# aask1357/hilcodec

Measured on AMD Instinct MI355X. Metric: audio-seconds/sec (xRT) encode+RVQ+decode, 24 kHz batch=256, higher is better.
Workload: dtype f32

## Files before the change

hilcodec_amd/csrc/resblock_kernel.h:

```cpp
#pragma once
#include "resblock_gemm.h"
#include "stream_gemm.h"

namespace {

struct Cols {
  long b;
  int t;
  int t_in;
  unsigned boff;
  unsigned hoff;
  int head, tail;
};
static_assert(sizeof(Cols) == 32, "no padding");

template <int C, bool STREAM, bool SCARRY = false, int NB = 1, bool W8 = false, int DRU = 0, bool POST = false, bool SPEC0 = false>
__global__ __launch_bounds__((Cfg<C, STREAM, SCARRY, NB, W8, DRU, POST, SPEC0>::NT), (Cfg<C, STREAM, SCARRY, NB, W8, DRU, POST, SPEC0>::MINW)) void resblock_kernel(ResArgs a) {
  using K = Cfg<C, STREAM, SCARRY, NB, W8, DRU, POST, SPEC0>;
  constexpr int DR = K::DR, UR = K::UR;
  using Pipe = WeightPipe<K>;
  constexpr int CBW = K::CBW, NW = K::NW, NT = K::NT, RW = K::RW, RB = K::RB, XS = K::XS, TO = K::TO, RSTEP = K::RSTEP;
  __shared__ __attribute__((aligned(16))) float Xbuf[4 + C * XS];
  constexpr bool DW_RELOAD = NB > 1 && K::NARROW && (4 + C * XS + NB * C * DWS) * 4 > 156 * 1024;
  __shared__ __attribute__((aligned(16))) float DW[(DW_RELOAD ? 1 : NB) * C * DWS];
// ... 80 lines not shown
      }
    } else {
    float tv[NB][RND][DWS];
#pragma unroll
    for (int q = 0; q < NB; ++q) {
      if (q < nblk) {
        const ResBlk& bq = a.blk[q];
#pragma unroll
        for (int it = 0; it < RND; ++it) {
          const int m = tid + it * NT;
          const int mc = (C % NT == 0 || m < C) ? m : C - 1;
#pragma unroll
          for (int j = 0; j < 5; ++j) tv[q][it][j] = bq.dw1_w[mc * 5 + j];
          tv[q][it][5] = bq.dw1_b[mc];
#pragma unroll
          for (int j = 0; j < 5; ++j) tv[q][it][6 + j] = bq.dw2_w[mc * 5 + j];
          tv[q][it][11] = bq.dw2_b[mc];
        }
      }
    }
#pragma unroll
    for (int q = 0; q < NB; ++q) {
      if (q < nblk) {
#pragma unroll
        for (int it = 0; it < RND; ++it) {
          const int m = tid + it * NT;
          if (C % NT == 0 || m < C) {
#pragma unroll
            for (int w4 = 0; w4 < DWS / 4; ++w4)
              *reinterpret_cast<f32x4*>(&DW[(q * C + m) * DWS + 4 * w4]) =
                  f32x4{tv[q][it][4 * w4], tv[q][it][4 * w4 + 1], tv[q][it][4 * w4 + 2], tv[q][it][4 * w4 + 3]};
          }
        }
      }
    }
    }
  }
  if constexpr (DR > 0 && !DWIDE) {
    constexpr int RND = (2 * C + NT - 1) / NT;
    float tw[RND][2 * DR + 1];
#pragma unroll
    for (int it = 0; it < RND; ++it) {
      const int m = tid + it * NT;
      const int mc = ((2 * C) % NT == 0 || m < 2 * C) ? m : 2 * C - 1;
#pragma unroll
      for (int j = 0; j < 2 * DR; ++j) tw[it][j] = a.dn.dw_w[mc * 2 * DR + j];
      tw[it][2 * DR] = a.dn.dw_b[mc];
    }
#pragma unroll
    for (int it = 0; it < RND; ++it) {
      const int m = tid + it * NT;
      if ((2 * C) % NT == 0 || m < 2 * C) {
#pragma unroll
        for (int j = 0; j < DDS; ++j) DWD[m * DDS + j] = j < 2 * DR ? tw[it][j] : (j == 8 ? tw[it][2 * DR] : 0.f);
      }
    }
  }
  if (tid < 4) Xbuf[tid] = 0.f;
  const int rsub = wave * K::RPI + (K::RPI > 1 ? lane / (K::NCOL / 4) : 0);
  const int c4 = (lane & (K::NCOL / 4 - 1)) * 4;
  [[maybe_unused]] const unsigned row_b = (unsigned)T * 4u;
  [[maybe_unused]] const bool one_head = STREAM && !K::NARROW && T >= K::NCOL;

  auto columns_of = [&](long tile) -> Cols {
    Cols s;
    s.boff = 0; s.hoff = 0; s.head = false; s.tail = false;
    if constexpr (STREAM) {
      const int flat = (int)tile * TO - K::HALO + c4;
      s.t_in = flat >= 0 && flat < a.B * T;
      const unsigned ub = s.t_in ? __umulhi((unsigned)flat, a.div_magic) >> a.div_shift : 0u;
      s.b = ub;
      s.t = s.t_in ? flat - (int)ub * T : 0;
      s.boff = (ub * (unsigned)(C * T) + (unsigned)s.t) * 4u;
      s.hoff = ub * (unsigned)(C * 4);
      s.head = s.t_in && s.t == 0;
      s.tail = s.t_in && c4 >= K::HALO && s.t == T - 4;
    } else {
      s.b = tile / a.tiles;
      s.t = (int)(tile - s.b * a.tiles) * TO + c4;
      s.t_in = s.t >= 0 && s.t < T;
    }
    return s;
  };
  auto xrow = [&](const Cols& s, int m) -> const f32x4* {
    if constexpr (STREAM)
      return reinterpret_cast<const f32x4*>(reinterpret_cast<const char*>(a.x) + (s.boff + (unsigned)m * row_b));
    else
      return reinterpret_cast<const f32x4*>(a.x + s.b * (long)C * T + (long)m * T + (s.t_in ? s.t : 0));
  };
  auto yrow = [&](const Cols& s, int m) -> f32x4* {
    if constexpr (STREAM)
      return reinterpret_cast<f32x4*>(reinterpret_cast<char*>(a.y) + (s.boff + (unsigned)m * row_b));
    else
      return reinterpret_cast<f32x4*>(a.y + s.b * (long)C * T + (long)m * T + s.t);
  };

  [[maybe_unused]] const float* hb0 = a.x;
  [[maybe_unused]] const float* hb1 = a.x;
  [[maybe_unused]] bool hv0 = false, hv1 = false;
  [[maybe_unused]] int blk_off = 0;
  Cols cs;
  const bool lane0 = c4 == 0, lane_last = c4 == K::NCOL - 4;
  auto prev_base = [&](int which) -> lptr_t {
    if constexpr (!K::CARRYMODE) return (lptr_t)(X + rsub * XS + c4 - 4);
    else return lane0 ? (lptr_t)(X + rsub * XS + K::NCOL + which * 4 + blk_off) : (lptr_t)(X + rsub * XS + c4 - 4);
  };
  auto prevs_of = [&](lptr_t pb, int m0, int which, f32x4 (&prev)[K::RB]) {
    if constexpr (!STREAM) {
#pragma unroll
      for (int i = 0; i < K::RB; ++i) prev[i] = *(lvec_t)(pb + i * RSTEP * XS);
    } else {
      bool staged = false;
      if constexpr (!K::NARROW) staged = one_head;
      if (staged) {
#pragma unroll
        for (int i = 0; i < K::RB; ++i) {
          const lptr_t pa = cs.head ? (lptr_t)(HS + (which * C + m0 + RSTEP * i) * 4) : pb + i * RSTEP * XS;
          prev[i] = *(lvec_t)pa;
        }
      } else {
        f32x4 hv[K::RB];
#pragma unroll
        for (int i = 0; i < K::RB; ++i)
          hv[i] = *reinterpret_cast<const f32x4*>((which ? hb1 : hb0) + ((which ? hv1 : hv0) ? cs.hoff + (unsigned)(m0 + RSTEP * i) * 4u : 0u));
#pragma unroll
        for (int i = 0; i < K::RB; ++i) {
          const f32x4 own = *(lvec_t)(pb + i * RSTEP * XS);
#pragma unroll
          for (int e = 0; e < 4; ++e) prev[i][e] = cs.head ? ((which ? hv1 : hv0) ? hv[i][e] : 0.f) : own[e];
        }
      }
    }
  };
  auto carry_out = [&](lptr_t xp, int which, const f32x4 (&cur)[K::RB]) {
    if constexpr (K::CARRYMODE) {
      if (lane_last) {
#pragma unroll
        for (int i = 0; i < K::RB; ++i) *(lvec_t)(xp + i * RSTEP * XS + 4 + which * 4 + blk_off) = cur[i];
      }
    }
  };

  float touch = 0.f;
  constexpr int LPR = K::NCOL / 32;
#ifdef HILC_RES_NO_UTOUCH
  constexpr bool UTOUCH = false;
#else
  constexpr bool UTOUCH = !STREAM && UR > 0 && !K::NARROW && (K::NCOL / (UR > 0 ? UR : 1)) % 32 == 0;
#endif
  constexpr int LPRU = UTOUCH ? K::NCOL / UR / 32 : 1;
  constexpr int NTOUCH = STREAM ? 1 : (UTOUCH ? (2 * C * LPRU + NT - 1) / NT : (C * LPR + NT - 1) / NT);
  float tv[NTOUCH];
#pragma unroll
  for (int i = 0; i < NTOUCH; ++i) tv[i] = 0.f;
  __shared__ long s_next;
  long run0 = blockIdx.x, run1 = a.total_tiles;
  long tile = blockIdx.x;
  if constexpr (K::CARRYMODE) {
    if (a.classes > 1) {
      const unsigned P = gridDim.x / (unsigned)a.classes, u = blockIdx.x % P, c = blockIdx.x / P;
      const long s0 = (long)u * a.total_tiles / P, len = (long)(u + 1) * a.total_tiles / P - s0;
      run0 = s0 + ((len * (long)a.cum[c]) >> 16);
      run1 = s0 + ((len * (long)a.cum[c + 1]) >> 16);
    } else if (a.run_tiles > 0) {
      run0 = (long)blockIdx.x * a.run_tiles;
      run1 = run0 + a.run_tiles < a.total_tiles ? run0 + a.run_tiles : a.total_tiles;
    } else {
      run0 = (long)blockIdx.x * a.total_tiles / gridDim.x;
      run1 = ((long)blockIdx.x + 1) * a.total_tiles / gridDim.x;
    }
    const bool mid = STREAM ? (run0 * TO) % T != 0 : run0 % a.tiles != 0;
    tile = (mid && run0 < run1) ? run0 - 1 : run0;
  }
  cs = columns_of(tile < run1 ? tile : 0);
  f32x4 xr[RW];
  if (UR == 0 && !SPEC0 && tile < run1) {
#pragma unroll
    for (int i = 0; i < RW; ++i) xr[i] = *xrow(cs, rsub + RSTEP * i);
  }
  lds_barrier();
  while (tile < run1) {
    const bool warm = K::CARRYMODE && tile < run0;
    constexpr bool TICKETS = !K::CARRYMODE && K::NW == 4;
    if constexpr (K::CARRYMODE && !STREAM) {
      if (tile % a.tiles == 0) {
        constexpr int NSLOT = 2 * NB + K::DCAR / 2 + (POST ? 1 : 0);
        for (int e = tid; e < NSLOT * C; e += NT)
          *reinterpret_cast<f32x4*>(X + (e / NSLOT) * XS + K::NCOL + (e % NSLOT) * 4) = f32x4{0.f, 0.f, 0.f, 0.f};
      }
    }
    if constexpr (!K::CARRYMODE) {
      if (TICKETS && a.sched != nullptr && tid == 0) s_next = (long)gridDim.x + atomicAdd(a.sched, 1);
    }
#if defined(HILC_DEBUG_WAVE_STAMPS)
    if (a.dbg != nullptr) {
      if (ws_base != nullptr && lane == 0) ws_base[(WS_MAXB - 1) * 3 + 1] = (unsigned long long)ws_k;
      ws_base = a.dbg + ((tile * NW + wave) * (long)WS_MAXB) * 3;
      if (lane == 0) { ws_base[(WS_MAXB - 1) * 3] = blockIdx.x; ws_base[(WS_MAXB - 1) * 3 + 2] = __builtin_amdgcn_s_memtime(); }
    }
    ws_k = 0;
#elif defined(HILC_DEBUG_STAMPS)
    stamp_tile = tile;
#endif
    STAMP(0);
    long next_tile = K::CARRYMODE ? tile + 1 : tile + gridDim.x;
    if constexpr (UR > 0) {
      const ResUp& up = a.up;
      const int Tin = T / UR;
      const int q0 = cs.t / UR, p0 = cs.t - q0 * UR;
      f32x16 acc[CBW];
#pragma unroll
      for (int i = 0; i < CBW; ++i)
#pragma unroll
        for (int r = 0; r < 16; ++r) acc[i][r] = 0.f;
#pragma nounroll
      for (int h = 0; h < 2; ++h) {
        const float* wu = (h ? up.w_hi : up.w_lo) + (long)wclass * (C * C / K::RH);
        asm volatile("" : "+s"(wu));
        {
          constexpr int UB = RW % 6 == 0 ? 6 : RB;
          constexpr bool UEXP = UR == 5;
          lptr_t xp = (lptr_t)(X + rsub * XS + c4);
          const bool has_prev = cs.t_in && q0 >= 1;
          [[maybe_unused]] const bool has_next = cs.t_in && q0 + 1 < Tin;
#pragma unroll
          for (int i0 = 0; i0 < RW; i0 += UB) {
            float xc[UB], xq[UB];
            [[maybe_unused]] float xn[UB];
            f32x4 wa[UB];
            [[maybe_unused]] f32x4 wb[UB];
#pragma unroll
            for (int i = 0; i < UB; ++i) {
              const int k = h * C + rsub + RSTEP * (i0 + i);
              const long row = (long)cs.b * (2 * C) + k;
              const float* xi = up.xin + (cs.t_in ? row * Tin + q0 : 0);
              xc[i] = xi[0];
              const float* pp = has_prev ? xi - 1 : (up.hist != nullptr && cs.t_in ? up.hist + row : xi);
              xq[i] = pp[0];
              if constexpr (UR == 2) {
                xn[i] = xi[cs.t_in ? 1 : 0];
                wa[i] = *reinterpret_cast<const f32x4*>(up.tr_w + k * 4);
              } else if constexpr (UEXP) {
                xn[i] = xi[has_next ? 1 : 0];
                const float* tw = up.tr_w + ((long)k * UR + p0) * 8;
                wa[i] = *reinterpret_cast<const f32x4*>(tw);
                wb[i] = *reinterpret_cast<const f32x4*>(tw + 4);
              } else {
                wa[i] = *reinterpret_cast<const f32x4*>(up.tr_w + k * (2 * UR) + p0);
                wb[i] = *reinterpret_cast<const f32x4*>(up.tr_w + k * (2 * UR) + UR + p0);
              }
            }
#pragma unroll
            for (int i = 0; i < UB; ++i) {
              const float a1 = prologue(xc[i], up.in_scale, 1);
              const float a0 = has_prev ? prologue(xq[i], up.in_scale, 1) : (up.hist != nullptr ? xq[i] : 0.f);
              f32x4 u;
              float a_last = a1;
              if constexpr (UR == 2) {
                const float a2 = prologue(xn[i], up.in_scale, 1);
                u[0] = fmaf(wa[i].x, a1, wa[i].z * a0);
                u[1] = fmaf(wa[i].y, a1, wa[i].w * a0);
                u[2] = fmaf(wa[i].x, a2, wa[i].z * a1);
                u[3] = fmaf(wa[i].y, a2, wa[i].w * a1);
                a_last = a2;
              } else if constexpr (UEXP) {
                const float a2 = has_next ? prologue(xn[i], up.in_scale, 1) : 0.f;
#pragma unroll
                for (int e = 0; e < 4; ++e) {
                  const bool nx = p0 + e >= UR;
                  u[e] = fmaf(wa[i][e], nx ? a2 : a1, wb[i][e] * (nx ? a1 : a0));
                }
                a_last = p0 + 3 >= UR ? a2 : a1;
              } else {
#pragma unroll
                for (int e = 0; e < 4; ++e) u[e] = fmaf(wa[i][e], a1, wb[i][e] * a0);
              }
              *(lvec_t)(xp + i * RSTEP * XS) = zero_unless(cs.t_in, u);
              if constexpr (STREAM) {
                if (cs.tail && !warm && up.hist_out != nullptr)
                  up.hist_out[(long)cs.b * (2 * C) + h * C + rsub + RSTEP * (i0 + i)] = a_last;
              }
            }
            xp += UB * RSTEP * XS;
            asm volatile("" : "+v"(xp));
            __builtin_amdgcn_sched_barrier(0);
          }
        }
        Pipe wp;
        wp.prefetch(wu, lane);
        lds_barrier();
        if constexpr (K::NARROW) gemm_phase_rolled<K, false>(wu, X, acc, wp, colblk, lane);
        else gemm_phase<K, false>(wu, X, acc, wp, colblk, lane);
        lds_barrier();
      }
      acc_to_x<K>(acc, X, rowblk0, colblk, lane);
      lds_barrier();
      {
        lptr_t xp = (lptr_t)(X + rsub * XS + c4);
#pragma unroll
        for (int i = 0; i < RW; ++i) {
          const float bv = up.bias != nullptr ? up.bias[rsub + RSTEP * i] : 0.f;
          f32x4 v = *(lvec_t)(xp + i * RSTEP * XS);
#pragma unroll
          for (int e = 0; e < 4; ++e) v[e] = up.bias != nullptr ? __fadd_rn(v[e], bv) : v[e];
          xr[i] = v;
        }
      }
      lds_barrier();
    }
    if constexpr (SPEC0) {
      const ResSpec0& sp = a.spec;
      constexpr int N = 64, NBIN = 33, SROWS = 40, KP0 = 4, DEPTH0 = 2;
      [[maybe_unused]] int split = K::NCOL;
      if constexpr (STREAM) {
        const int F0 = (int)tile * TO;
        const unsigned bA = __umulhi((unsigned)F0, a.div_magic) >> a.div_shift;
        const int tA0 = F0 - (int)bA * T;
        const int nxt = T - tA0;
        split = nxt < K::NCOL ? nxt : K::NCOL;
        const int lenA = (N - 1) + split;
        for (int i = tid; i < 2 * (N - 1) + K::NCOL; i += NT) {
          const bool second = i >= lenA;
          const unsigned b = bA + (second ? 1u : 0u);
          const int t = second ? i - lenA - (N - 1) : tA0 - (N - 1) + i;
          float v = 0.f;
          if (b < (unsigned)a.B) {
            if (t >= 0) v = sp.wav[(long)b * T + t];
            else if (sp.hist != nullptr && t >= -sp.hist_len) v = sp.hist[(long)b * sp.hist_len + sp.hist_len + t];
          }
          SEG[i] = v;
          SEGS[i] = v * sp.pre_in_scale;
        }
        for (int i = tid; i < (SROWS - NBIN) * 128; i += NT) X[(NBIN + (i >> 7)) * XS + (i & 127)] = 0.f;
      } else {
      const int f0 = cs.t - c4;
      {
        const int s0 = f0 - (N - 1);
        const float* wb = sp.wav + cs.b * (long)T;
        for (int i = tid; i < 127 + N; i += NT) {
          const int t = s0 + i;
          const float v = (t >= 0 && t < T) ? wb[t] : 0.f;
          SEG[i] = v;
          SEGS[i] = v * sp.pre_in_scale;
        }
        for (int i = tid; i < (SROWS - NBIN) * 128; i += NT) X[(NBIN + (i >> 7)) * XS + (i & 127)] = 0.f;
      }
      }
      lds_barrier();
      const int kh = lane >> 5, col = colblk * 32 + (lane & 31);
      const int colx = col + ((STREAM && col >= split) ? N - 1 : 0);
      f32x16 acc[CBW];
      {
        int off[8];
#pragma unroll
        for (int p = 0; p < 8; ++p) off[p] = colx + 2 * p + kh;
        auto bop = [&](int P) -> float { return SEG[off[P & 7] + 16 * (P >> 3)]; };
        stream_gemm<CBW, KP0, DEPTH0, N / 2 / KP0>(sp.dft, acc, lane, bop);
      }
      float nyq_im = 0.f;
#pragma unroll 8
      for (int k = 0; k < N; ++k) nyq_im = fmaf(sp.nyq[k], SEG[colx + k], nyq_im);
      const SpecFinish finish = SpecFinish::make(sp.mean, sp.stdv, sp.normalize);
#pragma unroll
      for (int i = 0; i < CBW; ++i) {
#pragma unroll
        for (int r = 0; r < 16; r += 2) {
          const int row = i * 32 + acc_row(r, lane);
          if (i == 0 && r == 0) {
            if (kh == 0) {
              X[0 * XS + col] = finish(acc[0][0], 0.f);
              X[(N / 2) * XS + col] = finish(acc[0][1], nyq_im);
            } else {
              X[(row >> 1) * XS + col] = finish(acc[0][0], acc[0][1]);
            }
          } else {
            X[(row >> 1) * XS + col] = finish(acc[i][r], acc[i][r + 1]);
          }
        }
      }
      lds_barrier();
      {
        const float* sl = X + kh * XS + col;
        auto bop = [&](int P) -> float { return sl[2 * P * XS]; };
        stream_gemm<CBW, KP0, DEPTH0, SROWS / 2 / KP0>(sp.pw, acc, lane, bop);
      }
      lds_barrier();
      acc_to_x<K>(acc, X, rowblk0, colblk, lane);
      lds_barrier();
      {
        lptr_t xp = (lptr_t)(X + rsub * XS + c4);
        float sm[8];
        const int c4x = c4 + ((STREAM && c4 >= split) ? N - 1 : 0);
#pragma unroll
        for (int j = 0; j < 8; ++j) sm[j] = SEGS[c4x + j + N - 5];
#pragma unroll
        for (int i = 0; i < RW; ++i) {
          const int m = rsub + RSTEP * i;
          const float bv = sp.bias != nullptr ? sp.bias[m] : 0.f;
          const float pb = sp.pre_b != nullptr ? sp.pre_b[m] : 0.f;
          float w5[5];
#pragma unroll
          for (int j = 0; j < 5; ++j) w5[j] = sp.pre_w[m * 5 + j];
          f32x4 v = *(lvec_t)(xp + i * RSTEP * XS);
#pragma unroll
          for (int e = 0; e < 4; ++e) {
            float acc5 = 0.f;
#pragma unroll
            for (int j = 0; j < 5; ++j) acc5 = fmaf(w5[j], sm[e + j], acc5);
            const float rr = sp.pre_b != nullptr ? __fadd_rn(acc5, pb) : acc5;
            float t = v[e];
            if (sp.bias != nullptr) t = __fadd_rn(t, bv);
            t = __fmul_rn(t, sp.out_scale);
            v[e] = __fadd_rn(t, rr);
          }
          xr[i] = v;
          if (i % 2 == 1) __builtin_amdgcn_sched_barrier(0);
        }
      }
      lds_barrier();
    }
#pragma nounroll
    for (int blk = 0; blk < nblk; ++blk) {
    const ResBlk& bp = a.blk[NB == 1 ? 0 : blk];
    const bool final_blk = NB == 1 || blk == nblk - 1;
    const bool last_blk = DR == 0 && !POST && final_blk;
    [[maybe_unused]] const bool post_blk = POST && final_blk;
    Cols cn = cs;
    bool have_next = false;
    if constexpr (NB > 1) blk_off = 8 * blk;
    const float* const DWb = DW + ((NB == 1 || DW_RELOAD) ? 0 : blk * C * DWS);
    if constexpr (DW_RELOAD) load_taps(bp, DW);
    if constexpr (STREAM) {
      hb0 = bp.hist1 != nullptr ? bp.hist1 : a.x;
      hb1 = bp.hist2 != nullptr ? bp.hist2 : a.x;
      hv0 = bp.hist1 != nullptr;
      hv1 = bp.hist2 != nullptr;
    }
    const float* w1t = bp.w1t + (long)wclass * (C * C / K::RH);
    const float* w2t = bp.w2t + (long)wclass * (C * C / K::RH);
    asm volatile("" : "+s"(w1t), "+s"(w2t));
    [[maybe_unused]] f32x4 hstage[(STREAM && !K::NARROW) ? (2 * C + NT - 1) / NT : 1];
    [[maybe_unused]] bool stage_hs = false;
    if constexpr (STREAM && !K::NARROW) {
      if (one_head) {
        const int first = (int)tile * TO - K::HALO, last = first + K::NCOL - 1;
        const unsigned bh = __umulhi((unsigned)last, a.div_magic) >> a.div_shift;
        const int hcol = (int)bh * T;
        stage_hs = hcol >= first && (int)bh < a.B;
        if (stage_hs) {
#pragma unroll
          for (int q = 0; q < (2 * C + NT - 1) / NT; ++q) {
            const int e = tid + q * NT;
            const int which = e >= C ? 1 : 0, m = e - which * C;
            f32x4 v = {0.f, 0.f, 0.f, 0.f};
            if (e < 2 * C && (which ? hv1 : hv0)) v = *reinterpret_cast<const f32x4*>((which ? hb1 : hb0) + bh * (unsigned)(C * 4) + (unsigned)m * 4u);
            hstage[q] = v;
          }
        }
      }
    }
    Pipe wp;
    wp.prefetch(w1t, lane);
    {
      lptr_t xp = (lptr_t)(X + rsub * XS + c4);
#pragma unroll
      for (int i0 = 0; i0 < RW; i0 += RB) {
#pragma unroll
        for (int i = 0; i < RB; ++i)
          *(lvec_t)(xp + i * RSTEP * XS) = prologue4v(zero_unless(cs.t_in, xr[i0 + i]), bp.pre_scale, 1);
        xp += RB * RSTEP * XS;
        asm volatile("" : "+v"(xp));
      }
    }
#pragma unroll
    for (int i = 0; i < NTOUCH; ++i) touch += tv[i];
    if constexpr (STREAM && !K::NARROW) {
      if (stage_hs) {
#pragma unroll
        for (int q = 0; q < (2 * C + NT - 1) / NT; ++q) {
          const int e = tid + q * NT;
          if (e < 2 * C) *reinterpret_cast<f32x4*>(&HS[e * 4]) = hstage[q];
        }
      }
    }
    lds_barrier();
    STAMP(1);
    if (TICKETS && a.sched != nullptr) next_tile = s_next;

    f32x16 acc[CBW];
    if constexpr (K::NARROW) gemm_phase_rolled<K>(w1t, X, acc, wp, colblk, lane);
    else gemm_phase<K>(w1t, X, acc, wp, colblk, lane);
    lds_barrier();
    STAMP(2);
    acc_to_x<K>(acc, X, rowblk0, colblk, lane);
    lds_barrier();
    STAMP(3);

    wp.prefetch(w2t, lane);
    lptr_t xp3 = (lptr_t)(X + rsub * XS + c4);
    lptr_t pb3 = prev_base(0);
#pragma unroll
    for (int i0 = 0; i0 < RW; i0 += RB) {
      f32x4 cur[RB], prev[RB], wa[RB];
      f32x2 wb[RB];
#pragma unroll
      for (int i = 0; i < RB; ++i) {
        const int m = rsub + RSTEP * (i0 + i);
        const lptr_t row = xp3 + i * RSTEP * XS;
        cur[i] = *(lvec_t)(row);
        wa[i] = *reinterpret_cast<const f32x4*>(&DWb[m * DWS]);
        wb[i] = *reinterpret_cast<const f32x2*>(&DWb[m * DWS + 4]);
      }
      prevs_of(pb3, rsub + RSTEP * i0, 0, prev);
      carry_out(xp3, 0, cur);
      if constexpr (STREAM) {
        if (cs.tail && !warm && bp.hist1_out != nullptr) {
#pragma unroll
          for (int i = 0; i < RB; ++i)
            *reinterpret_cast<f32x4*>(bp.hist1_out + cs.hoff + (rsub + RSTEP * (i0 + i)) * 4) = cur[i];
        }
      }
      f32x4 o[RB];
#pragma unroll
      for (int i = 0; i < RB; ++i) {
        const float v[8] = {prev[i].x, prev[i].y, prev[i].z, prev[i].w, cur[i].x, cur[i].y, cur[i].z, cur[i].w};
        const float w[5] = {wa[i].x, wa[i].y, wa[i].z, wa[i].w, wb[i].x};
#pragma unroll
        for (int e = 0; e < 4; ++e) {
          float s = 0.f;
#pragma unroll
          for (int j = 0; j < 5; ++j) s = fmaf(w[j], v[e + j], s);
          o[i][e] = elu_fast(__fadd_rn(s, wb[i].y));
        }
      }
#pragma unroll
      for (int i = 0; i < RB; ++i)
        *(lvec_t)(xp3 + i * RSTEP * XS) = o[i];
      xp3 += RB * RSTEP * XS;
      pb3 += RB * RSTEP * XS;
      asm volatile("" : "+v"(xp3), "+v"(pb3));
      __builtin_amdgcn_sched_barrier(0);
    }
    lds_barrier();
    STAMP(4);

    if constexpr (K::NARROW) gemm_phase_rolled<K>(w2t, X, acc, wp, colblk, lane);
    else gemm_phase<K>(w2t, X, acc, wp, colblk, lane);
    have_next = next_tile < run1;
    if (last_blk) cn = columns_of(have_next ? next_tile : tile);
    if constexpr (!STREAM && UR == 0 && !SPEC0) {
      if (final_blk) {
      long nb;
      int nt0;
      if constexpr (STREAM) {
        const int nf0 = (int)(have_next ? next_tile : tile) * TO - K::HALO;
        const unsigned q = __umulhi((unsigned)(nf0 < 0 ? 0 : nf0), a.div_magic) >> a.div_shift;
        nb = q;
        nt0 = nf0 - (int)q * T;
      } else {
        const long nt = have_next ? next_tile : tile;
        nb = nt / a.tiles;
        nt0 = (int)(nt - nb * a.tiles) * TO;
      }
      const float* nx = a.x + nb * (long)C * T;
#pragma unroll
      for (int i = 0; i < NTOUCH; ++i) {
        int e = tid + NT * i;
        e = e < C * LPR ? e : C * LPR - 1;
        int tt = nt0 + (e % LPR) * 32;
        tt = tt < 0 ? 0 : (tt > T - 1 ? T - 1 : tt);
        tv[i] = nx[(long)(e / LPR) * T + tt];
      }
      }
    }
    if constexpr (UTOUCH) {
      if (final_blk) {
        const long nt = have_next ? next_tile : tile;
        const long nb = nt / a.tiles;
        const int Tin = T / UR;
        const int nq0 = (int)(nt - nb * a.tiles) * TO / UR;
        const float* nx = a.up.xin + nb * (long)(2 * C) * Tin;
#pragma unroll
        for (int i = 0; i < NTOUCH; ++i) {
          int e = tid + NT * i;
          e = e < 2 * C * LPRU ? e : 2 * C * LPRU - 1;
          int ff = nq0 + (e % LPRU) * 32;
          ff = ff > Tin - 1 ? Tin - 1 : ff;
          tv[i] = nx[(long)(e / LPRU) * Tin + ff];
        }
      }
    }
    lds_barrier();
    STAMP(5);
    acc_to_x<K>(acc, X, rowblk0, colblk, lane);
    lds_barrier();
    STAMP(6);

    const bool out_ok = !warm && (STREAM ? (c4 >= K::HALO && cs.t_in) : cs.t < T);
    lptr_t xp6 = (lptr_t)(X + rsub * XS + c4);
    lptr_t pb6 = prev_base(1);
#pragma unroll
    for (int i0 = 0; i0 < RW; i0 += RB) {
      f32x4 cur[RB], prev[RB], wc[RB];
      f32x2 wb[RB];
#pragma unroll
      for (int i = 0; i < RB; ++i) {
        const int m = rsub + RSTEP * (i0 + i);
        const lptr_t row = xp6 + i * RSTEP * XS;
        cur[i] = *(lvec_t)(row);
        wb[i] = *reinterpret_cast<const f32x2*>(&DWb[m * DWS + 6]);
        wc[i] = *reinterpret_cast<const f32x4*>(&DWb[m * DWS + 8]);
      }
      prevs_of(pb6, rsub + RSTEP * i0, 1, prev);
      carry_out(xp6, 1, cur);
      if constexpr (STREAM) {
        if (cs.tail && !warm && bp.hist2_out != nullptr) {
#pragma unroll
          for (int i = 0; i < RB; ++i)
            *reinterpret_cast<f32x4*>(bp.hist2_out + cs.hoff + (rsub + RSTEP * (i0 + i)) * 4) = cur[i];
        }
      }
#pragma unroll
      for (int i = 0; i < RB; ++i) {
        const int m = rsub + RSTEP * (i0 + i);
        const float v[8] = {prev[i].x, prev[i].y, prev[i].z, prev[i].w, cur[i].x, cur[i].y, cur[i].z, cur[i].w};
        const float w[5] = {wb[i].x, wb[i].y, wc[i].x, wc[i].y, wc[i].z};
        f32x4 o;
#pragma unroll
        for (int e = 0; e < 4; ++e) {
          float s = 0.f;
#pragma unroll
          for (int j = 0; j < 5; ++j) s = fmaf(w[j], v[e + j], s);
          s = __fmul_rn(__fadd_rn(s, wc[i].w), bp.out_scale);
          o[e] = __fadd_rn(s, xr[i0 + i][e]);
        }
        if constexpr (NB == 1 && DR == 0 && !POST) {
          if (out_ok) *yrow(cs, m) = o;
        } else {
          if (last_blk) {
            if (out_ok) *yrow(cs, m) = o;
          } else if (post_blk) {
            *(lvec_t)(xp6 + i * RSTEP * XS) = prologue4v(o, a.post.in_scale, 1);
          } else {
            xr[i0 + i] = o;
          }
        }
      }
      if (UR == 0 && !SPEC0 && last_blk && have_next) {
#pragma unroll
        for (int i = 0; i < RB; ++i) xr[i0 + i] = *xrow(cn, rsub + RSTEP * (i0 + i));
      }
      xp6 += RB * RSTEP * XS;
      pb6 += RB * RSTEP * XS;
      asm volatile("" : "+v"(xp6), "+v"(pb6));
      __builtin_amdgcn_sched_barrier(0);
    }
    STAMP(7);
    lds_barrier();
    if (last_blk) cs = cn;
    }
    if constexpr (POST) {
      const bool have_next = next_tile < run1;
      const Cols cn = columns_of(have_next ? next_tile : tile);
      constexpr int PSLOT = K::NCOL + 8 * NB;
      float part[4] = {0.f, 0.f, 0.f, 0.f};
      lptr_t xq = (lptr_t)(X + rsub * XS + c4);
      lptr_t pq = lane0 ? (lptr_t)(X + rsub * XS + PSLOT) : (lptr_t)(X + rsub * XS + c4 - 4);
      const float* wq = a.post.w + rsub * 5;
      [[maybe_unused]] bool any_head = false;
      [[maybe_unused]] const float* hq = a.post.w;
      [[maybe_unused]] float* hqo = nullptr;
      [[maybe_unused]] bool qtail = false;
      if constexpr (STREAM) {
        const int first = (int)tile * TO, last = first + K::NCOL - 1;
        const unsigned bl = __umulhi((unsigned)last, a.div_magic) >> a.div_shift;
        any_head = (int)bl * T >= first || first % T == 0;
        if (a.post.hist != nullptr) hq = a.post.hist + cs.hoff + rsub * 4;
        qtail = cs.tail && !warm && a.post.hist_out != nullptr;
        if (a.post.hist_out != nullptr) hqo = a.post.hist_out + cs.hoff + rsub * 4;
      }
#pragma nounroll
      for (int i0 = 0; i0 < RW; i0 += RB) {
        f32x4 cur[RB], prev[RB];
        float w[RB][5];
#pragma unroll
        for (int i = 0; i < RB; ++i) {
          cur[i] = *(lvec_t)(xq + i * RSTEP * XS);
          prev[i] = *(lvec_t)(pq + i * RSTEP * XS);
#pragma unroll
          for (int j = 0; j < 5; ++j) w[i][j] = wq[i * RSTEP * 5 + j];
        }
        wq += RB * RSTEP * 5;
        if constexpr (STREAM) {
          if (any_head) {
            f32x4 hv[RB];
#pragma unroll
            for (int i = 0; i < RB; ++i)
              hv[i] = a.post.hist != nullptr ? *reinterpret_cast<const f32x4*>(hq + i * RSTEP * 4) : f32x4{0.f, 0.f, 0.f, 0.f};
#pragma unroll
            for (int i = 0; i < RB; ++i)
#pragma unroll
              for (int e = 0; e < 4; ++e) prev[i][e] = cs.head ? hv[i][e] : prev[i][e];
          }
          if (qtail) {
#pragma unroll
            for (int i = 0; i < RB; ++i) *reinterpret_cast<f32x4*>(hqo + i * RSTEP * 4) = cur[i];
          }
          hq += a.post.hist != nullptr ? RB * RSTEP * 4 : 0;
          hqo += RB * RSTEP * 4;
        }
        if (lane_last) {
#pragma unroll
          for (int i = 0; i < RB; ++i) *(lvec_t)(xq + i * RSTEP * XS + 4 + 8 * NB) = cur[i];
        }
#pragma unroll
        for (int i = 0; i < RB; ++i) {
          const float v[8] = {prev[i].x, prev[i].y, prev[i].z, prev[i].w, cur[i].x, cur[i].y, cur[i].z, cur[i].w};
#pragma unroll
          for (int e = 0; e < 4; ++e)
#pragma unroll
            for (int j = 0; j < 5; ++j) part[e] = fmaf(w[i][j], v[e + j], part[e]);
        }
        xq += RB * RSTEP * XS;
        pq += RB * RSTEP * XS;
        asm volatile("" : "+v"(xq), "+v"(pq));
        __builtin_amdgcn_sched_barrier(0);
      }
      *reinterpret_cast<f32x4*>(&PR[rsub * K::NCOL + c4]) = f32x4{part[0], part[1], part[2], part[3]};
      lds_barrier();
      if (tid < K::NCOL) {
        float sacc = PR[tid];
#pragma unroll
        for (int q = 1; q < POST_CLASSES; ++q) sacc = __fadd_rn(sacc, PR[q * K::NCOL + tid]);
        if (a.post.bias != nullptr) sacc = __fadd_rn(sacc, a.post.bias[0]);
        sacc = __fmul_rn(sacc, a.post.out_scale);
        if (a.post.do_tanh) sacc = tanhf(sacc);
        if constexpr (STREAM) {
          const long flat = (long)tile * TO + tid;
          if (!warm && flat < (long)a.B * T) a.post.wav[flat] = sacc;
        } else {
          const int t = cs.t - c4 + tid;
          if (!warm && t < T) a.post.wav[cs.b * (long)T + t] = sacc;
        }
      }
      cs = cn;
    }
    if constexpr (DR > 0) {
      const ResDown& dn = a.dn;
      const bool have_next = next_tile < run1;
      const Cols cn = columns_of(have_next ? next_tile : tile);
      const float* wd0 = dn.w_lo + (long)wclass * (C * C / K::RH);
      const float* wd1 = dn.w_hi + (long)wclass * (C * C / K::RH);
      asm volatile("" : "+s"(wd0), "+s"(wd1));
      Pipe wp;
      wp.prefetch(wd0, lane);
      auto d0 = [&]() {
        lptr_t xp = (lptr_t)(X + rsub * XS + c4);
#pragma unroll
        for (int i0 = 0; i0 < RW; i0 += RB) {
#pragma unroll
          for (int i = 0; i < RB; ++i)
            *(lvec_t)(xp + i * RSTEP * XS) = prologue4v(zero_unless(cs.t_in, xr[i0 + i]), dn.in_scale, 1);
          xp += RB * RSTEP * XS;
          asm volatile("" : "+v"(xp));
        }
      };
      d0();
      if (!DWIDE && !SPEC0 && have_next) {
#pragma unroll
        for (int i = 0; i < RW; ++i) xr[i] = *xrow(cn, rsub + RSTEP * i);
      }
      lds_barrier();
      f32x16 acc0[CBW];
      [[maybe_unused]] f32x16 acc1[DWIDE ? 1 : CBW];
      if constexpr (K::NARROW) gemm_phase_rolled<K>(wd0, X, acc0, wp, colblk, lane);
      else gemm_phase<K>(wd0, X, acc0, wp, colblk, lane);
      if constexpr (!DWIDE) {
        wp.prefetch(wd1, lane);
        if constexpr (K::NARROW) gemm_phase_rolled<K>(wd1, X, acc1, wp, colblk, lane);
        else gemm_phase<K>(wd1, X, acc1, wp, colblk, lane);
      }
      const bool out_ok = !warm && (STREAM ? cs.t_in : cs.t < T);
      [[maybe_unused]] const bool out_ok_tile = !warm;
      const int To = T / DR;
#pragma unroll
      for (int h = 0; h < 2; ++h) {
        if constexpr (DWIDE) {
          if (h == 1) {
            lds_barrier();
            wp.prefetch(wd1, lane);
            d0();
            if (have_next) {
#pragma unroll
              for (int i = 0; i < RW; ++i) xr[i] = *xrow(cn, rsub + RSTEP * i);
            }
            lds_barrier();
            gemm_phase_rolled<K>(wd1, X, acc0, wp, colblk, lane);
          }
        }
        lds_barrier();
        if constexpr (DWIDE) acc_to_x<K>(acc0, X, rowblk0, colblk, lane);
        else acc_to_x<K>(h ? acc1 : acc0, X, rowblk0, colblk, lane);
        lds_barrier();
        if constexpr (DWIDE) {
          constexpr int DC = K::DCAR;
          constexpr int DOFF = K::NCOL + 8 * NB;
          constexpr bool SLOTS = K::CARRYMODE;
          const int jl = c4 >> 2;
          const int t0 = STREAM ? (int)tile * TO : cs.t - c4;
          const int o = t0 / DR + jl;
          const int base = o * DR - DR - t0;
          [[maybe_unused]] unsigned sb = 0;
          int os = o;
          if constexpr (STREAM) {
            const bool in = o < a.B * To;
            sb = in ? __umulhi((unsigned)(o * DR), a.div_magic) >> a.div_shift : 0u;
            os = in ? o - (int)sb * To : 1;
          }
          [[maybe_unused]] const bool dhead = STREAM && os == 0;
          const bool act = out_ok_tile && (STREAM ? o < a.B * To : o < To) && o * DR + DR - 1 < t0 + K::NCOL;
          [[maybe_unused]] const int slot = DOFF + DC * h + DC;
          lptr_t rowp = (lptr_t)(X + rsub * XS);
          const float* wrow = dn.dw_w + (long)(h * C + rsub) * (2 * DR);
          const float* brow = dn.dw_b + (h * C + rsub);
          float wn[2 * DR], bn;
          [[maybe_unused]] float hn[STREAM ? DR : 1];
          [[maybe_unused]] const float* hrow = dn.dw_w;
          [[maybe_unused]] float* horow = nullptr;
          [[maybe_unused]] const bool use_hist = STREAM && dn.hist != nullptr;
          if constexpr (STREAM) {
            if (use_hist) hrow = dn.hist + ((long)sb * (2 * C) + h * C + rsub) * DR;
            if (dn.hist_out != nullptr) horow = dn.hist_out + ((long)cs.b * (2 * C) + h * C + rsub) * DR;
          }
// ... 103 lines not shown
          float bb[RB];
#pragma unroll
          for (int i = 0; i < RB; ++i) {
            const int m = h * C + rsub + RSTEP * (i0 + i);
            cur[i] = *(lvec_t)(xpd + i * RSTEP * XS);
            prev[i] = *(lvec_t)(pbd + i * RSTEP * XS);
            wa[i] = *reinterpret_cast<const f32x4*>(&DWD[m * DDS]);
            if constexpr (DR == 4) wb[i] = *reinterpret_cast<const f32x4*>(&DWD[m * DDS + 4]);
            bb[i] = DWD[m * DDS + 8];
          }
          if constexpr (STREAM) {
            const unsigned hro = (unsigned)cs.b * (unsigned)(2 * C * DR) + (unsigned)(h * C + rsub + RSTEP * i0) * DR;
#pragma unroll
            for (int i = 0; i < RB; ++i) {
              f32x4 hv = {0.f, 0.f, 0.f, 0.f};
              if (dn.hist != nullptr) {
                const float* hp = dn.hist + (cs.t_in ? hro + (unsigned)(RSTEP * i * DR) : 0u);
                if constexpr (DR == 4) hv = *reinterpret_cast<const f32x4*>(hp);
                else { const f32x2 h2 = *reinterpret_cast<const f32x2*>(hp); hv = f32x4{0.f, 0.f, h2.x, h2.y}; }
              }
#pragma unroll
              for (int e = 0; e < 4; ++e) prev[i][e] = cs.head ? hv[e] : prev[i][e];
            }
          }
          if (lane_last) {
#pragma unroll
            for (int i = 0; i < RB; ++i) *(lvec_t)(xpd + i * RSTEP * XS + 4 + 8 * NB + 4 * h) = cur[i];
          }
          if constexpr (STREAM) {
            if (cs.tail && !warm && dn.hist_out != nullptr) {
              const unsigned hro = (unsigned)cs.b * (unsigned)(2 * C * DR) + (unsigned)(h * C + rsub + RSTEP * i0) * DR;
#pragma unroll
              for (int i = 0; i < RB; ++i) {
                float* hp = dn.hist_out + hro + (unsigned)(RSTEP * i * DR);
                if constexpr (DR == 4) *reinterpret_cast<f32x4*>(hp) = cur[i];
                else *reinterpret_cast<f32x2*>(hp) = f32x2{cur[i].z, cur[i].w};
              }
            }
          }
#pragma unroll
          for (int i = 0; i < RB; ++i) {
            const int m = h * C + rsub + RSTEP * (i0 + i);
            const long yo = ((long)cs.b * (2 * C) + m) * (long)To + (cs.t_in ? cs.t / DR : 0);
            if constexpr (DR == 4) {
              const float v[8] = {prev[i].x, prev[i].y, prev[i].z, prev[i].w, cur[i].x, cur[i].y, cur[i].z, cur[i].w};
              const float w[8] = {wa[i].x, wa[i].y, wa[i].z, wa[i].w, wb[i].x, wb[i].y, wb[i].z, wb[i].w};
              float s0 = 0.f;
#pragma unroll
              for (int j = 0; j < 8; ++j) s0 = fmaf(w[j], v[j], s0);
              s0 = __fadd_rn(s0, bb[i]);
              if (out_ok) dn.y[yo] = dn.res != nullptr ? __fadd_rn(s0, dn.res[yo]) : s0;
            } else {
              const float v[6] = {prev[i].z, prev[i].w, cur[i].x, cur[i].y, cur[i].z, cur[i].w};
              const float w[4] = {wa[i].x, wa[i].y, wa[i].z, wa[i].w};
              f32x2 o2;
#pragma unroll
              for (int e = 0; e < 2; ++e) {
                float s0 = 0.f;
#pragma unroll
                for (int j = 0; j < 4; ++j) s0 = fmaf(w[j], v[2 * e + j], s0);
                o2[e] = __fadd_rn(s0, bb[i]);
              }
              if (out_ok) {
                if (dn.res != nullptr) {
                  const f32x2 r2 = *reinterpret_cast<const f32x2*>(dn.res + yo);
                  o2[0] = __fadd_rn(o2[0], r2.x);
                  o2[1] = __fadd_rn(o2[1], r2.y);
                }
                *reinterpret_cast<f32x2*>(dn.y + yo) = o2;
              }
            }
          }
          xpd += RB * RSTEP * XS;
          pbd += RB * RSTEP * XS;
          asm volatile("" : "+v"(xpd), "+v"(pbd));
          __builtin_amdgcn_sched_barrier(0);
        }
        }
      }
      lds_barrier();
      cs = cn;
    }
    tile = next_tile;
  }
  if (!K::CARRYMODE && K::NW == 4 && a.sched != nullptr && tid == 0) {
    if (atomicAdd(a.sched + 1, 1) == (int)gridDim.x - 1) {
      a.sched[0] = 0;
      a.sched[1] = 0;
    }
  }
  if (touch == 1.2345678e-30f) a.y[0] = touch;
#if defined(HILC_DEBUG_WAVE_STAMPS)
  if (ws_base != nullptr && lane == 0) ws_base[(WS_MAXB - 1) * 3 + 1] = (unsigned long long)ws_k;
#undef lds_barrier
#endif
#undef STAMP
}

}
```

Measured before the change: 3532.

## Walk tiles incrementally with uniform clip/tic counters and fast interior paths

```diff
diff --git a/hilcodec_amd/csrc/resblock_kernel.h b/hilcodec_amd/csrc/resblock_kernel.h
--- a/hilcodec_amd/csrc/resblock_kernel.h
+++ b/hilcodec_amd/csrc/resblock_kernel.h
@@ -186,6 +186,28 @@
     }
     return s;
   };
+  constexpr bool UWALK = !STREAM && C != 384;
+  [[maybe_unused]] int u_clip = 0, u_tic = 0, u_left = -1;
+  [[maybe_unused]] bool u_warm = false;
+  auto columns_at = [&](int clip, int tic) -> Cols {
+    Cols s;
+    s.boff = 0; s.hoff = 0; s.head = false; s.tail = false;
+    s.b = clip;
+    s.t = tic * TO + c4;
+    s.t_in = s.t < T;
+    return s;
+  };
+  auto next_pos = [&](bool have_next, int& nclip, int& ntic) {
+    const bool wrap = u_tic + 1 == a.tiles;
+    nclip = have_next ? (wrap ? u_clip + 1 : u_clip) : u_clip;
+    ntic = have_next ? (wrap ? 0 : u_tic + 1) : u_tic;
+  };
+  auto columns_next = [&](bool have_next) -> Cols {
+    int nclip, ntic;
+    next_pos(have_next, nclip, ntic);
+    return columns_at(nclip, ntic);
+  };
+  constexpr bool STEP_NEXT = UWALK && !(NB > 1 && DR == 0 && UR == 0 && !POST && !SPEC0);
   auto xrow = [&](const Cols& s, int m) -> const f32x4* {
     if constexpr (STREAM)
       return reinterpret_cast<const f32x4*>(reinterpret_cast<const char*>(a.x) + (s.boff + (unsigned)m * row_b));
@@ -276,18 +298,35 @@
     const bool mid = STREAM ? (run0 * TO) % T != 0 : run0 % a.tiles != 0;
     tile = (mid && run0 < run1) ? run0 - 1 : run0;
   }
-  cs = columns_of(tile < run1 ? tile : 0);
+  if constexpr (UWALK) {
+    const long first = tile < run1 ? tile : 0;
+    const long fclip = first / a.tiles;
+    u_clip = __builtin_amdgcn_readfirstlane((int)fclip);
+    u_tic = __builtin_amdgcn_readfirstlane((int)(first - fclip * a.tiles));
+    u_left = __builtin_amdgcn_readfirstlane(tile < run1 ? (int)(run1 - tile) - 1 : -1);
+    u_warm = __builtin_amdgcn_readfirstlane(tile < run0 ? 1 : 0) != 0;
+    cs = columns_at(u_clip, u_tic);
+  } else {
+    cs = columns_of(tile < run1 ? tile : 0);
+  }
   f32x4 xr[RW];
   if (UR == 0 && !SPEC0 && tile < run1) {
 #pragma unroll
     for (int i = 0; i < RW; ++i) xr[i] = *xrow(cs, rsub + RSTEP * i);
   }
   lds_barrier();
-  while (tile < run1) {
-    const bool warm = K::CARRYMODE && tile < run0;
+  while (UWALK ? u_left >= 0 : tile < run1) {
+    const bool warm = UWALK ? u_warm : (K::CARRYMODE && tile < run0);
+#ifdef HILC_RES_NO_INTERIOR
+    [[maybe_unused]] const bool tile_full = false;
+#elif defined(HILC_RES_COUNT_INTERIOR)
+    [[maybe_unused]] const bool tile_full = UWALK;
+#else
+    [[maybe_unused]] const bool tile_full = UWALK && (u_tic + 1) * K::NCOL <= T;
+#endif
     constexpr bool TICKETS = !K::CARRYMODE && K::NW == 4;
     if constexpr (K::CARRYMODE && !STREAM) {
-      if (tile % a.tiles == 0) {
+      if (UWALK ? u_tic == 0 : tile % a.tiles == 0) {
         constexpr int NSLOT = 2 * NB + K::DCAR / 2 + (POST ? 1 : 0);
         for (int e = tid; e < NSLOT * C; e += NT)
           *reinterpret_cast<f32x4*>(X + (e / NSLOT) * XS + K::NCOL + (e % NSLOT) * 4) = f32x4{0.f, 0.f, 0.f, 0.f};
@@ -312,6 +351,18 @@
       const ResUp& up = a.up;
       const int Tin = T / UR;
       const int q0 = cs.t / UR, p0 = cs.t - q0 * UR;
+      constexpr int UWS = UR == 2 ? 4 : (UR == 5 ? UR * 8 : 2 * UR);
+      const int lrow = rsub - wave * K::RPI;
+      [[maybe_unused]] const unsigned vx = ((unsigned)lrow * (unsigned)Tin + (unsigned)(q0 - 1)) * 4u;
+      [[maybe_unused]] const unsigned vw = (unsigned)(lrow * UWS + (UR == 2 ? 0 : (UR == 5 ? p0 * 8 : p0))) * 4u;
+#ifdef HILC_RES_COUNT_INTERIOR
+      [[maybe_unused]] const bool u_fast = UWALK;
+#elif defined(HILC_RES_NO_UFAST)
+      [[maybe_unused]] const bool u_fast = false;
+#else
+      [[maybe_unused]] const bool u_fast = tile_full && u_tic >= 1 && up.hist == nullptr &&
+                                           (UR != 5 || (u_tic * K::NCOL + K::NCOL - 4) / (UR > 0 ? UR : 1) + 1 < Tin);
+#endif
       f32x16 acc[CBW];
 #pragma unroll
       for (int i = 0; i < CBW; ++i)
@@ -321,20 +372,38 @@
       for (int h = 0; h < 2; ++h) {
         const float* wu = (h ? up.w_hi : up.w_lo) + (long)wclass * (C * C / K::RH);
         asm volatile("" : "+s"(wu));
-        {
+        auto build = [&](auto fast_c) __attribute__((always_inline)) {
+          constexpr bool FAST = decltype(fast_c)::value;
           constexpr int UB = RW % 6 == 0 ? 6 : RB;
           constexpr bool UEXP = UR == 5;
           lptr_t xp = (lptr_t)(X + rsub * XS + c4);
           const bool has_prev = cs.t_in && q0 >= 1;
           [[maybe_unused]] const bool has_next = cs.t_in && q0 + 1 < Tin;
+          [[maybe_unused]] const char* sx = reinterpret_cast<const char*>(up.xin + ((long)u_clip * (2 * C) + h * C + wave * K::RPI) * Tin);
+          [[maybe_unused]] const char* sw = reinterpret_cast<const char*>(up.tr_w + (h * C + wave * K::RPI) * UWS);
+          [[maybe_unused]] const size_t rsx = (size_t)(RSTEP * 4) * (size_t)Tin;
 #pragma unroll
           for (int i0 = 0; i0 < RW; i0 += UB) {
             float xc[UB], xq[UB];
             [[maybe_unused]] float xn[UB];
             f32x4 wa[UB];
             [[maybe_unused]] f32x4 wb[UB];
+            [[maybe_unused]] unsigned vxb = vx, vwb = vw;
+            if constexpr (FAST) asm volatile("" : "+v"(vxb), "+v"(vwb));
 #pragma unroll
             for (int i = 0; i < UB; ++i) {
+              if constexpr (FAST) {
+                const float* xi = reinterpret_cast<const float*>(sx + vxb);
+                const char* tw = sw + vwb + (i0 + i) * (RSTEP * UWS * 4);
+                xq[i] = xi[0];
+                xc[i] = xi[1];
+                if constexpr (UR == 2 || UEXP) xn[i] = xi[2];
+                wa[i] = *reinterpret_cast<const f32x4*>(tw);
+                if constexpr (UEXP) wb[i] = *reinterpret_cast<const f32x4*>(tw + 16);
+                else if constexpr (UR != 2) wb[i] = *reinterpret_cast<const f32x4*>(tw + UR * 4);
+                sx += rsx;
+                continue;
+              }
               const int k = h * C + rsub + RSTEP * (i0 + i);
               const long row = (long)cs.b * (2 * C) + k;
               const float* xi = up.xin + (cs.t_in ? row * Tin + q0 : 0);
@@ -357,7 +426,9 @@
 #pragma unroll
             for (int i = 0; i < UB; ++i) {
               const float a1 = prologue(xc[i], up.in_scale, 1);
-              const float a0 = has_prev ? prologue(xq[i], up.in_scale, 1) : (up.hist != nullptr ? xq[i] : 0.f);
+              float a0;
+              if constexpr (FAST) a0 = prologue(xq[i], up.in_scale, 1);
+              else a0 = has_prev ? prologue(xq[i], up.in_scale, 1) : (up.hist != nullptr ? xq[i] : 0.f);
               f32x4 u;
               float a_last = a1;
               if constexpr (UR == 2) {
@@ -368,7 +439,9 @@
                 u[3] = fmaf(wa[i].y, a2, wa[i].w * a1);
                 a_last = a2;
               } else if constexpr (UEXP) {
-                const float a2 = has_next ? prologue(xn[i], up.in_scale, 1) : 0.f;
+                float a2;
+                if constexpr (FAST) a2 = prologue(xn[i], up.in_scale, 1);
+                else a2 = has_next ? prologue(xn[i], up.in_scale, 1) : 0.f;
 #pragma unroll
                 for (int e = 0; e < 4; ++e) {
                   const bool nx = p0 + e >= UR;
@@ -379,7 +452,8 @@
 #pragma unroll
                 for (int e = 0; e < 4; ++e) u[e] = fmaf(wa[i][e], a1, wb[i][e] * a0);
               }
-              *(lvec_t)(xp + i * RSTEP * XS) = zero_unless(cs.t_in, u);
+              if constexpr (FAST) *(lvec_t)(xp + i * RSTEP * XS) = u;
+              else *(lvec_t)(xp + i * RSTEP * XS) = zero_unless(cs.t_in, u);
               if constexpr (STREAM) {
                 if (cs.tail && !warm && up.hist_out != nullptr)
                   up.hist_out[(long)cs.b * (2 * C) + h * C + rsub + RSTEP * (i0 + i)] = a_last;
@@ -388,6 +462,80 @@
             xp += UB * RSTEP * XS;
             asm volatile("" : "+v"(xp));
             __builtin_amdgcn_sched_barrier(0);
+          }
+        };
+        if constexpr (UWALK) {
+          if (u_fast) build(std::true_type{});
+          else build(std::false_type{});
+        } else {
+          {
+            constexpr int UB = RW % 6 == 0 ? 6 : RB;
+            constexpr bool UEXP = UR == 5;
+            lptr_t xp = (lptr_t)(X + rsub * XS + c4);
+            const bool has_prev = cs.t_in && q0 >= 1;
+            [[maybe_unused]] const bool has_next = cs.t_in && q0 + 1 < Tin;
+#pragma unroll
+            for (int i0 = 0; i0 < RW; i0 += UB) {
+              float xc[UB], xq[UB];
+              [[maybe_unused]] float xn[UB];
+              f32x4 wa[UB];
+              [[maybe_unused]] f32x4 wb[UB];
+#pragma unroll
+              for (int i = 0; i < UB; ++i) {
+                const int k = h * C + rsub + RSTEP * (i0 + i);
+                const long row = (long)cs.b * (2 * C) + k;
+                const float* xi = up.xin + (cs.t_in ? row * Tin + q0 : 0);
+                xc[i] = xi[0];
+                const float* pp = has_prev ? xi - 1 : (up.hist != nullptr && cs.t_in ? up.hist + row : xi);
+                xq[i] = pp[0];
+                if constexpr (UR == 2) {
+                  xn[i] = xi[cs.t_in ? 1 : 0];
+                  wa[i] = *reinterpret_cast<const f32x4*>(up.tr_w + k * 4);
+                } else if constexpr (UEXP) {
+                  xn[i] = xi[has_next ? 1 : 0];
+                  const float* tw = up.tr_w + ((long)k * UR + p0) * 8;
+                  wa[i] = *reinterpret_cast<const f32x4*>(tw);
+                  wb[i] = *reinterpret_cast<const f32x4*>(tw + 4);
+                } else {
+                  wa[i] = *reinterpret_cast<const f32x4*>(up.tr_w + k * (2 * UR) + p0);
+                  wb[i] = *reinterpret_cast<const f32x4*>(up.tr_w + k * (2 * UR) + UR + p0);
+                }
+              }
+#pragma unroll
+              for (int i = 0; i < UB; ++i) {
+                const float a1 = prologue(xc[i], up.in_scale, 1);
+                const float a0 = has_prev ? prologue(xq[i], up.in_scale, 1) : (up.hist != nullptr ? xq[i] : 0.f);
+                f32x4 u;
+                float a_last = a1;
+                if constexpr (UR == 2) {
+                  const float a2 = prologue(xn[i], up.in_scale, 1);
+                  u[0] = fmaf(wa[i].x, a1, wa[i].z * a0);
+                  u[1] = fmaf(wa[i].y, a1, wa[i].w * a0);
+                  u[2] = fmaf(wa[i].x, a2, wa[i].z * a1);
+                  u[3] = fmaf(wa[i].y, a2, wa[i].w * a1);
+                  a_last = a2;
+                } else if constexpr (UEXP) {
+                  const float a2 = has_next ? prologue(xn[i], up.in_scale, 1) : 0.f;
+#pragma unroll
+                  for (int e = 0; e < 4; ++e) {
+                    const bool nx = p0 + e >= UR;
+                    u[e] = fmaf(wa[i][e], nx ? a2 : a1, wb[i][e] * (nx ? a1 : a0));
+                  }
+                  a_last = p0 + 3 >= UR ? a2 : a1;
+                } else {
+#pragma unroll
+                  for (int e = 0; e < 4; ++e) u[e] = fmaf(wa[i][e], a1, wb[i][e] * a0);
+                }
+                *(lvec_t)(xp + i * RSTEP * XS) = zero_unless(cs.t_in, u);
+                if constexpr (STREAM) {
+                  if (cs.tail && !warm && up.hist_out != nullptr)
+                    up.hist_out[(long)cs.b * (2 * C) + h * C + rsub + RSTEP * (i0 + i)] = a_last;
+                }
+              }
+              xp += UB * RSTEP * XS;
+              asm volatile("" : "+v"(xp));
+              __builtin_amdgcn_sched_barrier(0);
+            }
           }
         }
         Pipe wp;
@@ -403,11 +551,25 @@
         lptr_t xp = (lptr_t)(X + rsub * XS + c4);
 #pragma unroll
         for (int i = 0; i < RW; ++i) {
-          const float bv = up.bias != nullptr ? up.bias[rsub + RSTEP * i] : 0.f;
-          f32x4 v = *(lvec_t)(xp + i * RSTEP * XS);
-#pragma unroll
-          for (int e = 0; e < 4; ++e) v[e] = up.bias != nullptr ? __fadd_rn(v[e], bv) : v[e];
-          xr[i] = v;
+          if constexpr (!UWALK) {
+            const float bv = up.bias != nullptr ? up.bias[rsub + RSTEP * i] : 0.f;
+            f32x4 v = *(lvec_t)(xp + i * RSTEP * XS);
+#pragma unroll
+            for (int e = 0; e < 4; ++e) v[e] = up.bias != nullptr ? __fadd_rn(v[e], bv) : v[e];
+            xr[i] = v;
+          } else {
+            xr[i] = *(lvec_t)(xp + i * RSTEP * XS);
+          }
+        }
+        if constexpr (UWALK) {
+          if (up.bias != nullptr) {
+#pragma unroll
+            for (int i = 0; i < RW; ++i) {
+              const float bv = up.bias[rsub + RSTEP * i];
+#pragma unroll
+              for (int e = 0; e < 4; ++e) xr[i][e] = __fadd_rn(xr[i][e], bv);
+            }
+          }
         }
       }
       lds_barrier();
@@ -567,13 +729,28 @@
     wp.prefetch(w1t, lane);
     {
       lptr_t xp = (lptr_t)(X + rsub * XS + c4);
-#pragma unroll
-      for (int i0 = 0; i0 < RW; i0 += RB) {
-#pragma unroll
-        for (int i = 0; i < RB; ++i)
-          *(lvec_t)(xp + i * RSTEP * XS) = prologue4v(zero_unless(cs.t_in, xr[i0 + i]), bp.pre_scale, 1);
-        xp += RB * RSTEP * XS;
-        asm volatile("" : "+v"(xp));
+#ifdef HILC_RES_NO_P0FAST
+      if (false) {
+#else
+      if (tile_full) {
+#endif
+#pragma unroll
+        for (int i0 = 0; i0 < RW; i0 += RB) {
+#pragma unroll
+          for (int i = 0; i < RB; ++i)
+            *(lvec_t)(xp + i * RSTEP * XS) = prologue4v(xr[i0 + i], bp.pre_scale, 1);
+          xp += RB * RSTEP * XS;
+          asm volatile("" : "+v"(xp));
+        }
+      } else {
+#pragma unroll
+        for (int i0 = 0; i0 < RW; i0 += RB) {
+#pragma unroll
+          for (int i = 0; i < RB; ++i)
+            *(lvec_t)(xp + i * RSTEP * XS) = prologue4v(zero_unless(cs.t_in, xr[i0 + i]), bp.pre_scale, 1);
+          xp += RB * RSTEP * XS;
+          asm volatile("" : "+v"(xp));
+        }
       }
     }
 #pragma unroll
@@ -650,8 +827,11 @@
 
     if constexpr (K::NARROW) gemm_phase_rolled<K>(w2t, X, acc, wp, colblk, lane);
     else gemm_phase<K>(w2t, X, acc, wp, colblk, lane);
-    have_next = next_tile < run1;
-    if (last_blk) cn = columns_of(have_next ? next_tile : tile);
+    have_next = UWALK ? u_left > 0 : next_tile < run1;
+    if (last_blk) {
+      if constexpr (STEP_NEXT) cn = columns_next(have_next);
+      else cn = columns_of(have_next ? next_tile : tile);
+    }
     if constexpr (!STREAM && UR == 0 && !SPEC0) {
       if (final_blk) {
       long nb;
@@ -662,9 +842,16 @@
         nb = q;
         nt0 = nf0 - (int)q * T;
       } else {
-        const long nt = have_next ? next_tile : tile;
-        nb = nt / a.tiles;
-        nt0 = (int)(nt - nb * a.tiles) * TO;
+        if constexpr (STEP_NEXT) {
+          int nclip, ntic;
+          next_pos(have_next, nclip, ntic);
+          nb = nclip;
+          nt0 = ntic * TO;
+        } else {
+          const long nt = have_next ? next_tile : tile;
+          nb = nt / a.tiles;
+          nt0 = (int)(nt - nb * a.tiles) * TO;
+        }
       }
       const float* nx = a.x + nb * (long)C * T;
 #pragma unroll
@@ -679,10 +866,11 @@
     }
     if constexpr (UTOUCH) {
       if (final_blk) {
-        const long nt = have_next ? next_tile : tile;
-        const long nb = nt / a.tiles;
+        int nclip, ntic;
+        next_pos(have_next, nclip, ntic);
+        const long nb = nclip;
         const int Tin = T / UR;
-        const int nq0 = (int)(nt - nb * a.tiles) * TO / UR;
+        const int nq0 = ntic * TO / UR;
         const float* nx = a.up.xin + nb * (long)(2 * C) * Tin;
 #pragma unroll
         for (int i = 0; i < NTOUCH; ++i) {
@@ -764,8 +952,8 @@
     if (last_blk) cs = cn;
     }
     if constexpr (POST) {
-      const bool have_next = next_tile < run1;
-      const Cols cn = columns_of(have_next ? next_tile : tile);
+      const bool have_next = UWALK ? u_left > 0 : next_tile < run1;
+      const Cols cn = [&]() -> Cols { if constexpr (STEP_NEXT) return columns_next(have_next); else return columns_of(have_next ? next_tile : tile); }();
       constexpr int PSLOT = K::NCOL + 8 * NB;
       float part[4] = {0.f, 0.f, 0.f, 0.f};
       lptr_t xq = (lptr_t)(X + rsub * XS + c4);
@@ -851,8 +1039,8 @@
     }
     if constexpr (DR > 0) {
       const ResDown& dn = a.dn;
-      const bool have_next = next_tile < run1;
-      const Cols cn = columns_of(have_next ? next_tile : tile);
+      const bool have_next = UWALK ? u_left > 0 : next_tile < run1;
+      const Cols cn = [&]() -> Cols { if constexpr (STEP_NEXT) return columns_next(have_next); else return columns_of(have_next ? next_tile : tile); }();
       const float* wd0 = dn.w_lo + (long)wclass * (C * C / K::RH);
       const float* wd1 = dn.w_hi + (long)wclass * (C * C / K::RH);
       asm volatile("" : "+s"(wd0), "+s"(wd1));
@@ -1122,6 +1310,13 @@
       cs = cn;
     }
     tile = next_tile;
+    if constexpr (UWALK) {
+      const bool wrap = u_tic + 1 == a.tiles;
+      u_tic = wrap ? 0 : u_tic + 1;
+      u_clip = wrap ? u_clip + 1 : u_clip;
+      --u_left;
+      u_warm = false;
+    }
   }
   if (!K::CARRYMODE && K::NW == 4 && a.sched != nullptr && tid == 0) {
     if (atomicAdd(a.sched + 1, 1) == (int)gridDim.x - 1) {
```

After: 3544 (median of 6 runs). Within noise of the previous version (+0.3%).
